# HumaticsLAB/SEAM-Match-RCNN

Hardware: AMD Instinct MI355X
Metric: video-clips/sec (10f x 800^2, 32 ROI/f, 1k gallery) (higher is better)
Workload: dtype f32; 1 GPU; configs[1] full pipeline, fixed ROIs: 10 frames 800x800 -> ResNet-50-FPN + RPN head -> RoIAlign 14x14 (32 ROI/frame) -> mask head -> match trunk x2 -> SEAM NLB + attention pool (32 seq x 10) -> pair logits vs 1000-product bank -> top-20; hip_graph=False, hip_streams=2, frames=10, rois_per_frame=32, gallery=1000, topk=20, parallelism=single GPU

## Files before the change

include/seam_hip.h:

```cpp
#ifndef SEAM_HIP_H
#define SEAM_HIP_H

#include <stdint.h>

#ifdef __cplusplus
extern "C" {
#endif

typedef void* seam_stream_t;

int seam_version(void);
int seam_fastdiv_exact(unsigned d, unsigned long long n_max);
const char* seam_error_string(int code);

int seam_option_count(void);
const char* seam_option_name(int index);
int seam_set_option(const char* name, int value);
int seam_get_option(const char* name, int* value);

int seam_conv_kred(int C, int R, int S);
int seam_conv_rows_padded(int K);
int seam_conv_tile(int M, int K);
int seam_conv_tile_prec(int prec, int M, int K);
int seam_conv_tile_taps(int prec, int M, int K, int taps);
// ... 7 lines not shown
                    int relu, seam_stream_t stream);

int seam_conv2d_upres_f32(const float* x, const float* w_packed, const float* scale, const float* shift,
                          const float* top, float* y, int N, int H, int W, int C, int K, int R, int S,
                          int stride, int pad, int Ht, int Wt, int relu, seam_stream_t stream);

int seam_conv2d_crop_f32(const float* x, const float* w_packed, const float* scale, const float* shift, float* y,
                         int N, int H, int W, int C, int K, int R, int S, int stride, int pad, int Ho, int Wo,
                         int relu, seam_stream_t stream);
int seam_conv2d_crop_f16(const void* x, const void* w_packed, const float* scale, const float* shift, void* y,
                         int N, int H, int W, int C, int K, int R, int S, int stride, int pad, int Ho, int Wo,
                         int relu, seam_stream_t stream);

int seam_conv2d_dual_f32(const float* x1, const float* x2, const float* w_packed, const float* scale,
                         const float* shift, float* y, int N, int Ho, int Wo, int C1, int H2, int W2, int C2,
                         int stride2, int K, int relu, seam_stream_t stream);

int seam_conv1x1_sw_config(int M, int C1, int C2, int K);
int seam_conv1x1_sw_f32(const float* x, const float* x2, const float* w, const float* shift, const float* residual, float* y,
                        int M, int C1, int C2, int K, int relu, int res_mode, int Ho, int Wo, int rH, int rW,
                        seam_stream_t stream);

int seam_conv1x1_f16pc_supported(long long M, int C, int K);
long long seam_conv1x1_f16pc_weight_halves(int K, int C);
int seam_pack_conv1x1_weight_f16pc(const float* w, void* w_packed, int K, int C, seam_stream_t stream);
int seam_conv1x1_f16pc(const void* x, const void* w_packed, const float* scale, const float* shift, const void* residual, void* y,
                       long long M, int C, int K, int relu, seam_stream_t stream);

int seam_conv1x1_sxpc_supported(long long M, int C, int K);
long long seam_conv1x1_sxpc_weight_bytes(int K, int C);
int seam_pack_conv1x1_weight_sxpc(const float* w, void* w_packed, int K, int C, seam_stream_t stream);
int seam_conv1x1_sxpc(const float* x, const void* w_packed, const float* scale, const float* shift, const float* residual, float* y,
                      long long M, int C, int K, int relu, seam_stream_t stream);

int seam_conv1x1_swh_config(long long M, int C1, int C2, int K);
int seam_conv1x1_swh_f16(const void* x, const void* x2, const void* w, const float* scale, const float* shift,
                         const void* residual, void* y, long long M, int C1, int C2, int K, int relu, int res_mode,
                         int Ho, int Wo, int rH, int rW, seam_stream_t stream);

int seam_stem_s2d_swh_f16(const void* xpad, const void* w, const float* scale, const float* shift, void* y, int N, int Ho, int Wo,
                          int relu, seam_stream_t stream);

int seam_conv1x1_pc_supported(long long M, int C, int K);
long long seam_conv1x1_pc_weight_floats(int K, int C);
int seam_pack_conv1x1_pc_f32(const float* w, float* w_packed, int K, int C, seam_stream_t stream);
int seam_conv1x1_pc_f32(const float* x, const float* w_packed, const float* scale, const float* shift, const float* residual,
                        float* y, long long M, int C, int K, int relu, seam_stream_t stream);

int seam_conv2d_dual_f16(const void* x1, const void* x2, const void* w_packed, const float* scale,
                         const float* shift, void* y, int N, int Ho, int Wo, int C1, int H2, int W2, int C2,
                         int stride2, int K, int relu, seam_stream_t stream);

int seam_conv_kred_f16(int C, int R, int S);
int seam_pack_conv_weight_f16(const float* w, void* w_packed, int K, int Cin, int R, int S,
                              int Cstore, int mode, seam_stream_t stream);
int seam_conv2d_f16(const void* x, const void* w_packed, const float* scale, const float* shift,
                    const void* residual, void* y, int N, int H, int W, int C, int K, int R, int S,
                    int stride, int pad, int relu, int y_f32, seam_stream_t stream);

int seam_preprocess_f32(const float* img, float* out, int in_h, int in_w, int out_h, int out_w,
                        int Hp, int Wp, seam_stream_t stream);

int seam_preprocess_f16(const float* img, void* out , int in_h, int in_w, int out_h,
                        int out_w, int Hp, int Wp, seam_stream_t stream);

int seam_preprocess_batch_f32(const float* imgs, size_t img_stride, float* out, int n, int in_h, int in_w,
// ... 341 lines not shown
```

seam-match-rcnn_amd/_native.py:

```python
from __future__ import annotations

import ctypes as C
import os

import torch

_HERE = os.path.dirname(os.path.abspath(__file__))
LIB_PATH = os.environ.get("SEAM_LIB_PATH") or os.path.join(_HERE, "lib", "libseam_hip.so")

_p = C.c_void_p
_i = C.c_int
_f = C.c_float
_i64 = C.c_int64

class TrunkLayer(C.Structure):
    _fields_ = [("w", C.c_void_p), ("u", C.c_void_p), ("u24", C.c_void_p), ("scale", C.c_void_p), ("shift", C.c_void_p)]


SGD_MAX_SLOTS = 32
SGD_FP_SLOTS = 64


class SgdTensor(C.Structure):
    _fields_ = [("p", C.c_void_p), ("g", C.c_void_p), ("buf", C.c_void_p), ("numel", C.c_int64), ("group", C.c_int), ("reserved", C.c_int)]
# ... 30 lines not shown
    "seam_set_option": (_i, [C.c_char_p, _i]),
    "seam_get_option": (_i, [C.c_char_p, C.POINTER(_i)]),
    "seam_conv_kred": (_i, [_i, _i, _i]),
    "seam_conv_rows_padded": (_i, [_i]),
    "seam_conv_tile": (_i, [_i, _i]),
    "seam_conv_tile_prec": (_i, [_i, _i, _i]),
    "seam_conv_tile_taps": (_i, [_i, _i, _i, _i]),
    "seam_pack_conv_weight_f32": (_i, [_p, _p, _i, _i, _i, _i, _i, _i, _p]),
    "seam_conv2d_f32": (_i, [_p, _p, _p, _p, _p, _p, _i, _i, _i, _i, _i, _i, _i, _i, _i, _i, _p]),
    "seam_linear_narrow_supported": (_i, [_i, _i]),
    "seam_pack_linear_narrow_f32": (_i, [_p, _p, _i, _i, _p]),
    "seam_linear_narrow_f32": (_i, [_p, _p, _p, _p, C.c_longlong, _i, _i, _i, _p]),
    "seam_conv2d_crop_f32": (_i, [_p, _p, _p, _p, _p, _i, _i, _i, _i, _i, _i, _i, _i, _i, _i, _i, _i, _p]),
    "seam_conv2d_crop_f16": (_i, [_p, _p, _p, _p, _p, _i, _i, _i, _i, _i, _i, _i, _i, _i, _i, _i, _i, _p]),
    "seam_preprocess_s2d_batch_f32": (_i, [_p, C.c_size_t, _p, _i, _i, _i, _i, _i, _i, _i, _p]),
    "seam_preprocess_s2d_batch_f16": (_i, [_p, C.c_size_t, _p, _i, _i, _i, _i, _i, _i, _i, _p]),
    "seam_preprocess_s2d_pad_batch_f16": (_i, [_p, C.c_size_t, _p, _i, _i, _i, _i, _i, _i, _i, _i, _i, _p]),
    "seam_conv2d_dual_f32": (_i, [_p, _p, _p, _p, _p, _p, _i, _i, _i, _i, _i, _i, _i, _i, _i, _i, _p]),
    "seam_conv1x1_pc_supported": (_i, [C.c_longlong, _i, _i]),
    "seam_conv1x1_pc_weight_floats": (C.c_longlong, [_i, _i]),
    "seam_pack_conv1x1_pc_f32": (_i, [_p, _p, _i, _i, _p]),
    "seam_conv1x1_pc_f32": (_i, [_p, _p, _p, _p, _p, _p, C.c_longlong, _i, _i, _i, _p]),
    "seam_conv1x1_sw_config": (_i, [_i, _i, _i, _i]),
    "seam_conv1x1_sw_f32": (_i, [_p, _p, _p, _p, _p, _p, _i, _i, _i, _i, _i, _i, _i, _i, _i, _i, _p]),
    "seam_conv1x1_swh_config": (_i, [C.c_longlong, _i, _i, _i]),
    "seam_conv1x1_f16pc_supported": (_i, [C.c_longlong, _i, _i]),
    "seam_conv1x1_f16pc_weight_halves": (C.c_longlong, [_i, _i]),
    "seam_pack_conv1x1_weight_f16pc": (_i, [_p, _p, _i, _i, _p]),
    "seam_conv1x1_f16pc": (_i, [_p, _p, _p, _p, _p, _p, C.c_longlong, _i, _i, _i, _p]),
    "seam_conv1x1_sxpc_supported": (_i, [C.c_longlong, _i, _i]),
    "seam_conv1x1_sxpc_weight_bytes": (C.c_longlong, [_i, _i]),
    "seam_pack_conv1x1_weight_sxpc": (_i, [_p, _p, _i, _i, _p]),
    "seam_conv1x1_sxpc": (_i, [_p, _p, _p, _p, _p, _p, C.c_longlong, _i, _i, _i, _p]),
    "seam_conv1x1_swh_f16": (_i, [_p, _p, _p, _p, _p, _p, _p, C.c_longlong, _i, _i, _i, _i, _i, _i, _i, _i, _i, _p]),
    "seam_stem_s2d_swh_f16": (_i, [_p, _p, _p, _p, _p, _i, _i, _i, _i, _p]),
    "seam_conv2d_dual_f16": (_i, [_p, _p, _p, _p, _p, _p, _i, _i, _i, _i, _i, _i, _i, _i, _i, _i, _p]),
    "seam_conv2d_upres_f32": (_i, [_p, _p, _p, _p, _p, _p, _i, _i, _i, _i, _i, _i, _i, _i, _i, _i, _i, _i, _p]),
    "seam_pack_conv_weight_bx3": (_i, [_p, _p, _p, _i, _i, _i, _i, _i, _i, _p]),
    "seam_conv2d_bx3": (_i, [_p, _p, _p, _p, _p, _p, _i, _i, _i, _i, _i, _i, _i, _i, _i, _i, _p]),
    "seam_pack_conv_weight_sx": (_i, [_p, _p, _p, _i, _i, _i, _i, _i, _i, _p]),
    "seam_conv2d_sx": (_i, [_p, _p, _p, _p, _p, _p, _i, _i, _i, _i, _i, _i, _i, _i, _i, _i, _i, _p]),
    "seam_wino_supported": (_i, [_i, _i, _i, _i, _i]),
    "seam_wino_weight_floats": (C.c_longlong, [_i, _i]),
    "seam_wino_slot_fill_pct": (_i, [_i, _i, _i, _i, _i, _i]),
    "seam_wino_tile_variant": (_i, [_i, _i, _i, _i, _i, _i]),
    "seam_pack_conv_weight_wino_f32": (_i, [_p, _p, _i, _i, _i, _i, _p]),
    "seam_wino_issue_slots": (C.c_longlong, [_i, _i, _i, _i, _i, _i]),
    "seam_wino24_issue_slots": (C.c_longlong, [_i, _i, _i, _i, _i, _i]),
    "seam_wino24_variant": (_i, [_i, _i, _i, _i, _i, _i]),
    "seam_wino24_form": (_i, [_i, _i, _i, _i, _i, _i]),
    "seam_wino24_weight_floats": (C.c_longlong, [_i, _i]),
    "seam_pack_conv_weight_wino24_f32": (_i, [_p, _p, _i, _i, _i, _i, _p]),
    "seam_conv3x3_wino24_f32": (_i, [_p, _p, _p, _p, _p, _p, _i, _i, _i, _i, _i, _i, _i, _p]),
    "seam_conv3x3_wino_f32": (_i, [_p, _p, _p, _p, _p, _p, _i, _i, _i, _i, _i, _i, _i, _p]),
    "seam_conv3x3_f16pc_supported": (_i, [_i, _i, _i, _i, _i, _i]),
    "seam_conv3x3_f16pc_pays": (_i, [_i, _i, _i, _i, _i, _i]),
    "seam_f16pc_weight_halves": (C.c_longlong, [_i, _i]),
    "seam_pack_conv_weight_f16pc": (_i, [_p, _p, _i, _i, _i, _p]),
    "seam_conv3x3_f16pc": (_i, [_p, _p, _p, _p, _p, _p, _i, _i, _i, _i, _i, _i, _i, _p]),
    "seam_conv_kred_f16": (_i, [_i, _i, _i]),
    "seam_pack_conv_weight_f16": (_i, [_p, _p, _i, _i, _i, _i, _i, _i, _p]),
    "seam_conv2d_f16": (_i, [_p, _p, _p, _p, _p, _p, _i, _i, _i, _i, _i, _i, _i, _i, _i, _i, _i, _p]),
    "seam_preprocess_f32": (_i, [_p, _p, _i, _i, _i, _i, _i, _i, _p]),
    "seam_preprocess_batch_f32": (_i, [_p, C.c_size_t, _p, _i, _i, _i, _i, _i, _i, _i, _p]),
    "seam_preprocess_batch_f16": (_i, [_p, C.c_size_t, _p, _i, _i, _i, _i, _i, _i, _i, _p]),
    "seam_preprocess_u8": (_i, [_p, _p, _i, _i, _i, _i, _i, _i, _i, _p]),
# ... 168 lines not shown
```

seam-match-rcnn_amd/csrc/seam_pwsx.hip:

```cpp
#include <hip/hip_runtime.h>
#include "seam_device.h"
#include <stdint.h>
#include <type_traits>
#include "seam_fastdiv.h"
#include "seam_launch.h"
#include "seam_pack_items.h"
#include "seam_split.h"

namespace {

constexpr int BM = 128;
constexpr int CK = 64;
constexpr int KS = CK / 16;
constexpr int PLB = CK * 2;
constexpr int ROWB = 3 * PLB + 16;
constexpr int ABUF = BM * ROWB;
constexpr int NP = BM * (CK / 4) / 256;
constexpr int TROW = 128 + 16;
constexpr int TBUF = 32 * TROW;
constexpr int TR0 = 2 * ABUF;
constexpr int LDS_BYTES = TR0 + 4 * 2 * TBUF;
static_assert(LDS_BYTES <= 160 * 1024 && ABUF + 3 * PLB < 65536 && 4 * 32 * ROWB < 65536, "LDS map / ds immediates");
constexpr int RB = 4;
static_assert(RB == KS, "ring slot = k-step of the chunk");
constexpr int RVA = 3;

#ifndef SEAM_SXPC_ABL
#define SEAM_SXPC_ABL 0
#endif

struct SxpcArgs {
    const float* x;
    const void* w;
    const float* scale;
    const float* shift;
    const float* res;
    float* y;
    int M, C, K, relu;
    int tiles_n, nchunks, total_tiles;
    unsigned m_tiles_n;
};

__global__ __launch_bounds__(512, 2) void conv1x1_sxpc(const SxpcArgs p) {
    extern __shared__ __attribute__((aligned(16))) char smem[];
    const int tid = threadIdx.x, lane = tid & 63;
    const int wave = __builtin_amdgcn_readfirstlane(tid >> 6);
    const bool consumer = wave < 4;
    const int n = p.nchunks;

    const XcdTiles xt = xcd_tiles(p.total_tiles);
    const int ntiles = xt.ntiles, S = xt.stride;
    if (ntiles == 0) return;
    const int tile0 = xt.tile0();
    const size_t row_bytes = (size_t)p.C * 4, out_row = (size_t)p.K * 4;
    const int total_chunks = ntiles * n;

    if (!consumer) {
        const int ptid = tid - 256;
        unsigned goff[NP];
        LDSQ char* lp[NP];
#pragma unroll
        for (int r = 0; r < NP; ++r) {
            const int row = (ptid >> 4) + 16 * r;
            goff[r] = (unsigned)(row * p.C * 4 + (ptid & 15) * 16);
            lp[r] = (LDSQ char*)smem + row * ROWB + (ptid & 15) * 8;
        }
        f32x4 rq[2][NP];
        int tile = tile0, ck = 0, tiles_left = ntiles;
        auto x_desc = [&](const int tl) {
            const int tm = fdivu(tl, p.tiles_n, p.m_tiles_n);
            const int row0 = tm * BM;
            const int rows = tiles_left > 0 ? min(BM, p.M - row0) : 0;
            return __builtin_amdgcn_make_buffer_rsrc((void*)((const char*)p.x + (size_t)(tiles_left > 0 ? row0 : 0) * row_bytes), 0,
                                                     (int)(rows * row_bytes), 0x00020000);
        };
        __amdgpu_buffer_rsrc_t rs = x_desc(tile);
        auto request = [&](f32x4 (&dst)[NP]) {
#pragma unroll
            for (int r = 0; r < NP; ++r)
                dst[r] = __builtin_bit_cast(f32x4, __builtin_amdgcn_raw_buffer_load_b128(rs, (SEAM_SXPC_ABL & 1) ? kOob : goff[r], ck * (CK * 4), 0));
            if (++ck == n) {
                ck = 0;
                tile += S;
                --tiles_left;
                rs = x_desc(tile);
            }
        };
        auto store_chunk = [&](const f32x4 (&src)[NP], const int buf) {
            if (SEAM_SXPC_ABL & 1) return;
#pragma unroll
            for (int r = 0; r < NP; ++r) {
                u32x2 q0, q1, q2;
                if (SEAM_SXPC_ABL & 4) {
                    q0[0] = __builtin_bit_cast(unsigned, src[r][0]); q0[1] = __builtin_bit_cast(unsigned, src[r][1]);
                    q1[0] = __builtin_bit_cast(unsigned, src[r][2]); q1[1] = __builtin_bit_cast(unsigned, src[r][3]); q2 = q0;
                } else {
                    split3_bf16(src[r], q0, q1, q2);
                }
                *reinterpret_cast<u32x2 LDSQ*>(lp[r] + buf * ABUF) = q0;
                *reinterpret_cast<u32x2 LDSQ*>(lp[r] + buf * ABUF + PLB) = q1;
                *reinterpret_cast<u32x2 LDSQ*>(lp[r] + buf * ABUF + 2 * PLB) = q2;
            }
        };
        request(rq[0]);
        request(rq[1]);
        store_chunk(rq[0], 0);
        request(rq[0]);
        LDS_BAR();
        for (int c = 0; c < total_chunks; c += 2) {
            store_chunk(rq[1], 1);
            request(rq[1]);
            LDS_BAR();
            if (c + 1 >= total_chunks) break;
            store_chunk(rq[0], 0);
            request(rq[0]);
            LDS_BAR();
        }
    } else {
// ... 119 lines not shown
                }
                auto put = [&](const int m) {
#pragma unroll
                    for (int qd = 0; qd < 4; ++qd)
                        *reinterpret_cast<f32x4 LDSQ*>(tw + (m & 1) * TBUF + qd * 32) =
                            f32x4{acc[m][4 * qd], acc[m][4 * qd + 1], acc[m][4 * qd + 2], acc[m][4 * qd + 3]};
                };
                put(0);
#pragma unroll
                for (int m = 0; m < 4; ++m) {
                    if (m + 1 < 4) put(m + 1);
#pragma unroll
                    for (int i = 0; i < 4; ++i) {
                        f32x4 v = *reinterpret_cast<const f32x4 LDSQ*>(tr + (m & 1) * TBUF + i * (8 * TROW));
                        v = v * sc + sh;
                        if (RES) v += rv[m][i];
                        if (RELU) {
#pragma unroll
                            for (int e = 0; e < 4; ++e) v[e] = fmaxf(v[e], 0.f);
                        }
                        __builtin_amdgcn_raw_buffer_store_b128(__builtin_bit_cast(u32x4, v), y_rsrc, ocol + m * K32 + i * K8, 0, 0);
                    }
                }
            };
            if (p.res) {
                if (p.relu) finish_tile(std::true_type{}, std::true_type{}); else finish_tile(std::true_type{}, std::false_type{});
            } else {
                if (p.relu) finish_tile(std::false_type{}, std::true_type{}); else finish_tile(std::false_type{}, std::false_type{});
            }
        }
    }
}

__global__ void sxpc_pack_kernel(const float* __restrict__ w, unsigned short* __restrict__ out, int K, int C) {
    const size_t total = (size_t)K * C / 8;
    for (size_t i = (size_t)blockIdx.x * blockDim.x + threadIdx.x; i < total; i += (size_t)gridDim.x * blockDim.x)
        seam_pack::sxpc_item(w, out, i, C);
}

int sxpc_plan(SxpcArgs& a, long long M, int C, int K) {
    if (M <= 0 || C < 256 || (C % CK) || K < 128 || (K % 128)) return 1;
    if ((unsigned long long)BM * C * 4 >= kOob || (unsigned long long)BM * K * 4 >= kOob) return 1;
    if ((unsigned long long)(C / 16) * 3072 >= kOob) return 1;
    const long long tiles_m = (M + BM - 1) / BM;
    const long long total = tiles_m * (K / 128);
    if (total >= (1LL << 24) || M >= (1LL << 31)) return 1;
    a.M = (int)M; a.C = C; a.K = K;
    a.tiles_n = K / 128; a.nchunks = C / CK; a.total_tiles = (int)total;
    if (!seam_fastdiv::exact(a.tiles_n, 2ull * total + (1ull << 16))) return 1;
    a.m_tiles_n = seam_fastdiv::magic(a.tiles_n);
    return 0;
}

}

extern "C" {

int seam_conv1x1_sxpc_supported(long long M, int C, int K) {
    SxpcArgs a;
    return sxpc_plan(a, M, C, K) == 0 ? 1 : 0;
}

long long seam_conv1x1_sxpc_weight_bytes(int K, int C) { return (long long)K * C * 6; }

int seam_pack_conv1x1_weight_sxpc(const float* w, void* w_packed, int K, int C, void* stream) {
    SxpcArgs a;
    if (sxpc_plan(a, 1, C, K)) return (int)hipErrorInvalidValue;
    const size_t total = (size_t)K * C / 8;
    const unsigned grid = seam_launch::grid256(total);
    hipLaunchKernelGGL(sxpc_pack_kernel, dim3(grid), dim3(256), 0, (hipStream_t)stream, w, (unsigned short*)w_packed, K, C);
    return (int)hipGetLastError();
}

int seam_conv1x1_sxpc(const float* x, const void* w_packed, const float* scale, const float* shift, const float* residual, float* y,
                      long long M, int C, int K, int relu, void* stream) {
    SxpcArgs a;
    if ((relu != 0 && relu != 1) || sxpc_plan(a, M, C, K)) return (int)hipErrorInvalidValue;
    a.x = x; a.w = w_packed; a.scale = scale; a.shift = shift; a.res = residual; a.y = y; a.relu = relu;
    int ncu;
    const hipError_t e = seam_launch::prepare<conv1x1_sxpc>(LDS_BYTES, &ncu);
    if (e != hipSuccess) return (int)e;
    const unsigned grid = (unsigned)(a.total_tiles > ncu ? ncu : a.total_tiles);
    hipLaunchKernelGGL(conv1x1_sxpc, dim3(grid), dim3(512), LDS_BYTES, (hipStream_t)stream, a);
    return (int)hipGetLastError();
}

}
```

seam-match-rcnn_amd/models/detection.py:

```python
from __future__ import annotations

import math
from collections import OrderedDict
from typing import List, Sequence, Tuple

import numpy as np
import torch
import torch.nn.functional as F
from torch import nn

from .. import ops

RESNET50_LAYERS = ((3, 64, 1), (4, 128, 2), (6, 256, 2), (3, 512, 2))
BBOX_XFORM_CLIP = math.log(1000.0 / 16)
NMS_MAX_BOXES = 16384


import os as _os


def _key(params, dtype=None) -> tuple:
    return tuple((p.data_ptr(), p._version) for p in params) + (dtype,)


def cdt(module):
    return getattr(module, "compute_dtype", torch.float32)


def adt(module) -> torch.dtype:
    return torch.float16 if cdt(module) == torch.float16 else torch.float32


SPLIT_F32 = _os.environ.get("SEAM_SPLIT_F32", "1") != "0"
SPLIT_DTYPE = {"6": ops.SX6, "9": ops.SX9}[_os.environ.get("SEAM_SPLIT_TERMS", "6")]
SPLIT_C3_MIN_C = 256
SPLIT_CLASSES = frozenset(c for c in _os.environ.get("SEAM_SPLIT_CLASSES", "c1,c3,c2s2").split(",") if c)


def split_on(module) -> bool:
    return (SPLIT_F32 and getattr(module, "split_f32", True) and cdt(module) == torch.float32 and not module.training
            and not torch.is_grad_enabled())


def set_split_f32(model: nn.Module, on: bool) -> nn.Module:
    for m in model.modules():
        m.split_f32 = bool(on)
    return model


def set_compute_dtype(model: nn.Module, dtype) -> nn.Module:
    if dtype not in (torch.float32, torch.float16, ops.BX3):
        raise ValueError('compute dtype must be torch.float32, torch.float16 or "bf16x3"')
    for m in model.modules():
        m.compute_dtype = dtype
    return model


def resized_size(h: int, w: int, min_size: int = 800, max_size: int = 1333) -> Tuple[int, int, float]:
    scale = min(float(min_size) / float(min(h, w)), float(max_size) / float(max(h, w)))
    return int(math.floor(float(h) * scale)), int(math.floor(float(w) * scale)), scale


class PreparedImages:

    def __init__(self, tensor, sizes, orig, padded, min_size, max_size, size_divisible, s2d):
        self.tensor, self.sizes, self.orig, self.padded = tensor, list(sizes), list(orig), tuple(padded)
        self.min_size, self.max_size, self.size_divisible, self.s2d = min_size, max_size, size_divisible, bool(s2d)

    def __len__(self):
# ... 101 lines not shown
        return self._all()

    def _pack_key(self):
        dt = cdt(self)
        return _key(self._all(), dt) + (dt == torch.float32 and SPLIT_F32 and getattr(self, "split_f32", True),)

    def packed(self):
        dt = cdt(self)
        sx = dt == torch.float32 and SPLIT_F32 and getattr(self, "split_f32", True)
        key = self._pack_key()
        if self._pk is None or key != self._pk_key:
            with torch.no_grad():
                pk = {"stem": ops.pack_conv(self.conv1.weight, None, self.bn1.tensors(), stride=2, pad=3,
                                            cstore=8 if dt == torch.float16 else 4, bn_eps=self.bn1.eps, dtype=dt)}
                if dt in (torch.float32, torch.float16):
                    def s2d_weight():
                        w8 = F.pad(self.conv1.weight.detach().to(torch.float32), (1, 0, 1, 0))
                        return w8.view(64, 3, 4, 2, 4, 2).permute(0, 3, 5, 1, 2, 4).reshape(64, 12, 4, 4).contiguous()
                    ws = ops.derived_source(s2d_weight, (self.conv1.weight,))
                    pk["stem_s2d"] = ops.pack_conv(ws, None, self.bn1.tensors(), stride=1, pad=2, cstore=12 if dt == torch.float32 else 16,
                                                   bn_eps=self.bn1.eps, wino=False, dtype=dt)
                    if dt == torch.float16 and STEM_SWH:
                        pk["stem_rows"] = F.pad(ws, (0, 0, 0, 0, 0, 4)).permute(0, 2, 3, 1).reshape(64, 256).to(torch.float16).contiguous()
                for li in range(1, 5):
                    for bi, b in enumerate(getattr(self, f"layer{li}")):
                        e = {"c1": ops.pack_conv(b.conv1.weight, None, b.bn1.tensors(), bn_eps=b.bn1.eps, dtype=dt),
                             "c2": ops.pack_conv(b.conv2.weight, None, b.bn2.tensors(), stride=b.stride, pad=1,
                                                 bn_eps=b.bn2.eps, dtype=dt),
                             "c3": ops.pack_conv(b.conv3.weight, None, b.bn3.tensors(), bn_eps=b.bn3.eps, dtype=dt)}
                        if b.downsample is not None:
                            e["ds"] = ops.pack_conv(b.downsample[0].weight, None, b.downsample[1].tensors(),
                                                    stride=b.stride, bn_eps=b.downsample[1].eps, dtype=dt)
                            if dt in (torch.float32, torch.float16) and FUSE_SHORTCUT:
                                e["c3ds"] = ops.pack_conv_dual(b.conv3.weight, b.bn3.tensors(), b.downsample[0].weight,
                                                               b.downsample[1].tensors(), bn_eps=b.bn3.eps, dtype=dt)
                        if sx:
                            if "c1" in SPLIT_CLASSES:
                                e["c1x"] = ops.pack_conv(b.conv1.weight, None, b.bn1.tensors(), bn_eps=b.bn1.eps, dtype=SPLIT_DTYPE)
                            if "c2s2" in SPLIT_CLASSES and b.stride == 2:
                                e["c2x"] = ops.pack_conv(b.conv2.weight, None, b.bn2.tensors(), stride=2, pad=1, bn_eps=b.bn2.eps,
                                                         dtype=SPLIT_DTYPE)
                            if "c3" in SPLIT_CLASSES and "c3ds" not in e and b.conv3.in_channels >= SPLIT_C3_MIN_C:
                                e["c3x"] = ops.pack_conv(b.conv3.weight, None, b.bn3.tensors(), bn_eps=b.bn3.eps, dtype=SPLIT_DTYPE)
                        pk[(li, bi)] = e
            self._pk, self._pk_key = pk, key
        return self._pk

    def forward(self, x: torch.Tensor, s2d_padded: bool = False, taped: bool = False) -> List[torch.Tensor]:
        if taped:
            return self.forward_taped(x, s2d_padded)
        pk = self.packed()
        n = x.shape[0]
        if BODY_STREAMS >= 2 and n >= 2 * BODY_STREAMS and x.is_cuda:
            cur = torch.cuda.current_stream()
            if (getattr(self, "_streams", None) is None or len(self._streams) != BODY_STREAMS
                    or self._streams[0].device != x.device):
                self._streams = [torch.cuda.Stream(device=x.device) for _ in range(BODY_STREAMS)]
            spad = 3 if s2d_padded else 0
            h1, w1 = ((x.shape[1] - spad, x.shape[2] - spad) if x.shape[-1] in (12, 16) else
                      ((x.shape[1] + 6 - 7) // 2 + 1, (x.shape[2] + 6 - 7) // 2 + 1))
            hh, ww = (h1 + 2 - 3) // 2 + 1, (w1 + 2 - 3) // 2 + 1
            outs = []
            for li, (nblk, planes, stride) in enumerate(RESNET50_LAYERS, start=1):
                if stride == 2:
                    hh, ww = (hh - 1) // 2 + 1, (ww - 1) // 2 + 1
                outs.append(torch.empty((n, hh, ww, planes * 4), dtype=x.dtype, device=x.device))
            bounds = [n * i // BODY_STREAMS for i in range(BODY_STREAMS + 1)]
            for i, st in enumerate(self._streams):
# ... 1 lines not shown
                with torch.cuda.stream(st):
                    lo, hi = bounds[i], bounds[i + 1]
                    self._run(x[lo:hi], pk, [o[lo:hi] for o in outs], s2d_padded)
            for st in self._streams:
                cur.wait_stream(st)
            return outs
        return self._run(x, pk, None, s2d_padded)

    def _stem(self, x, pk, s2d_padded=False, pool=True):
        if x.shape[-1] in (12, 16):
            streaming = ("stem_rows" in pk and x.dtype == torch.float16 and x.shape[-1] == 16
                         and (x.shape[1] - (3 if s2d_padded else 0)) * (x.shape[2] - (3 if s2d_padded else 0)) >= 128)
            if s2d_padded and not streaming:
                x = x[:, 2:-1, 2:-1].contiguous()
            if streaming:
                x = ops.stem_s2d_f16(x, pk["stem_rows"], pk["stem_s2d"].scale, pk["stem_s2d"].shift, relu=True, padded=s2d_padded)
            else:
                x = ops.conv2d(x, pk["stem_s2d"], relu=True, out_hw=(x.shape[1], x.shape[2]))
        else:
            x = ops.conv2d(x, pk["stem"], relu=True)
        return ops.maxpool2d(x, 3, 2, 1) if pool else x

    def _run(self, x, pk, outs, s2d_padded=False):
        x = self._stem(x, pk, s2d_padded)
        sx = split_on(self)
        feats = []
        for li in range(1, 5):
            nblk = len(getattr(self, f"layer{li}"))
            for bi in range(nblk):
                e = pk[(li, bi)]
                o = ops.conv2d(x, e.get("c1x", e["c1"]) if sx else e["c1"], relu=True)
                o = ops.conv2d(o, e.get("c2x", e["c2"]) if sx else e["c2"], relu=True)
                if "c3ds" in e:
                    x = ops.conv2d_dual(o, x, e["c3ds"], getattr(self, f"layer{li}")[bi].stride, relu=True)
                    continue
                idt = ops.conv2d(x, e["ds"]) if "ds" in e else x
                x = ops.conv2d(o, e.get("c3x", e["c3"]) if sx else e["c3"], relu=True, residual=idt,
                               out=outs[li - 1] if (outs is not None and bi == nblk - 1) else None)
            feats.append(x)
        return feats

    def blocks(self):
        return [(li, bi, b) for li in range(1, 5) for bi, b in enumerate(getattr(self, f"layer{li}"))]

    def forward_taped(self, x: torch.Tensor, s2d_padded: bool = False) -> List[torch.Tensor]:
        from ..autograd import BodyFunction
        if cdt(self) != torch.float32 or x.dtype != torch.float32:
            raise NotImplementedError("the training branch of the ResNet body is fp32 only: call set_compute_dtype(torch.float32)")
        stem = self.conv1.weight.requires_grad
        if stem and not self.train_stem:
            raise NotImplementedError(
                "ResNet body training: the stem of the backbone (backbone.body.conv1 and its max-pool) has no backward; freeze "
                "it with `model.backbone.body.conv1.weight.requires_grad_(False)` or build the model with "
                "trainable_backbone_layers <= 4 (layer1..layer4 may learn).  Stem training is opt-in: set `train_stem=True` "
                "(constructor keyword, or the attribute of backbone.body).")
        pk = self.packed()
        blocks = self.blocks()
        if stem:
            weights = [self.conv1.weight] + [w for _, _, b in blocks for w in block_weights(b)]
            meta = [(pk[(li, bi)], b.stride, b.downsample is not None, bi == len(getattr(self, f"layer{li}")) - 1) for li, bi, b in blocks]
            stem_fwd = (lambda f: self._stem(f, pk, s2d_padded, pool=False), pk["stem"].scale)
            return list(BodyFunction.apply(meta, stem_fwd, x, *weights))
        start = next((i for i, (_, _, b) in enumerate(blocks) if any(p.requires_grad for p in b.parameters())), len(blocks))
        with torch.no_grad():
            x = self._stem(x.detach(), pk, s2d_padded)
            feats = []
            for li, bi, b in blocks[:start]:
# ... 559 lines not shown
```

seam-match-rcnn_amd/ops.py:

```python
from __future__ import annotations

import ctypes as C
import functools
from dataclasses import dataclass
from typing import Optional, Sequence

import torch

from . import _native

F32 = torch.float32
F16 = torch.float16


def _stream() -> int:
    return torch.cuda.current_stream().cuda_stream


def _req(t: torch.Tensor, dtype=F32, name: str = "tensor") -> torch.Tensor:
    if not isinstance(t, torch.Tensor) or not t.is_cuda:
        raise _native.SeamNativeError(f"{name}: expected a tensor on the HIP device (no CPU path exists)")
    if dtype is not None and t.dtype != dtype:
        raise TypeError(f"{name}: expected {dtype}, got {t.dtype}")
    return t if t.is_contiguous() else t.contiguous()
# ... 577 lines not shown
    x, top = _req(x, F32, "x"), _req(top, F32, "top")
    n, h, w, c = x.shape
    if c != pc.Cstore:
        raise ValueError(f"conv2d_topdown: input has {c} channels, weights packed for {pc.Cstore}")
    ho = (h + 2 * pc.pad - pc.R) // pc.stride + 1
    wo = (w + 2 * pc.pad - pc.S) // pc.stride + 1
    if top.dim() != 4 or top.shape[0] != n or top.shape[3] != pc.K:
        raise ValueError("conv2d_topdown: top must be NHWC [N,Ht,Wt,K]")
    y = torch.empty((n, ho, wo, pc.K), dtype=F32, device=x.device)
    lib = _native.lib()
    sw = _sw_ok(pc, h, w) and h * w >= 64
    tr = CONV_TRACE is not None and _trace_begin(
        _sw_variant(lib, "sw", n * h * w, c, pc.K) if sw else _igemm_variant(lib, F32, n * ho * wo, pc.K),
        2.0 * n * ho * wo * pc.K * pc.R * pc.S * (pc.Cin or pc.Cstore), (n, h, w, c, pc.K, pc.R, pc.stride),
        float(4 * (x.numel() + pc.w.numel() + y.numel() + top.numel())))
    if sw:
        _sw_launch(lib, x, None, pc, top, y, n * h * w, c, 0, False, 2, ho, wo, top.shape[1], top.shape[2])
    else:
        _native.check(lib.seam_conv2d_upres_f32(_ptr(x), _ptr(pc.w), _ptr(pc.scale), _ptr(pc.shift), _ptr(top), _ptr(y),
                                                n, h, w, c, pc.K, pc.R, pc.S, pc.stride, pc.pad, top.shape[1], top.shape[2], 0,
                                                _stream()), "seam_conv2d_upres_f32")
    if tr:
        _trace_end(tr)
    return y


def pack_conv_dual(w1: torch.Tensor, bn1, w2: torch.Tensor, bn2, bn_eps: float = 1e-5, dtype=F32) -> PackedConv:
    def fold(w, bn):
        bw, bb, rm, rv = (t.detach().to(F32) for t in bn)
        sc = bw * torch.rsqrt(rv + bn_eps)
        return w.detach().to(F32).reshape(w.shape[0], -1) * sc[:, None], bb - rm * sc
    w = derived_source(lambda: torch.cat([fold(w1, bn1)[0], fold(w2, bn2)[0]], 1).contiguous(), (w1, w2))
    shift = derived_source(lambda: (fold(w1, bn1)[1] + fold(w2, bn2)[1]).contiguous(), ())
    return pack_conv(w[:, :, None, None], shift, wino=False, dtype=dtype)


def conv2d_dual(x1: torch.Tensor, x2: torch.Tensor, pc: PackedConv, stride2: int = 1, relu: bool = False) -> torch.Tensor:
    x1 = _req(x1, None, "x1")
    if pc.dtype not in (F32, F16) or pc.R != 1 or pc.S != 1:
        raise ValueError("conv2d_dual: needs fp32 / fp16 1x1 weights from pack_conv_dual")
    dt = pc.dtype
    x1, x2 = _req(x1, dt, "x1"), _req(x2, dt, "x2")
    n, ho, wo, c1 = x1.shape
    n2, h2, w2, c2 = x2.shape
    cm = 32 if dt == F32 else 64
    if n2 != n or c1 + c2 != pc.Cstore or c1 % cm or c2 % cm:
        raise ValueError(f"conv2d_dual: channel / batch mismatch (C1, C2 must be multiples of {cm} and sum to the packed width)")
    if (ho - 1) * stride2 >= h2 or (wo - 1) * stride2 >= w2:
        raise ValueError("conv2d_dual: x2 too small for the output grid")
    y = torch.empty((n, ho, wo, pc.K), dtype=dt, device=x1.device)
    lib = _native.lib()
    same = stride2 == 1 and (h2, w2) == (ho, wo)
    sw = dt == F32 and same and _sw_ok(pc, ho, wo)
    swh = dt == F16 and same and _swh_ok(pc, ho, wo) and lib.seam_conv1x1_swh_config(n * ho * wo, c1, c2, pc.K) != 0
    tr = CONV_TRACE is not None and _trace_begin(
        _sw_variant(lib, "sw" if sw else "swh", n * ho * wo, c1 + c2, pc.K) if sw or swh else _igemm_variant(lib, dt, n * ho * wo, pc.K, dual=True),
        2.0 * n * ho * wo * pc.K * (c1 + c2), (n, ho, wo, c1 + c2, pc.K, 1, 1),
        float(x1.element_size() * (x1.numel() + n * ho * wo * c2 + pc.w.numel() + y.numel())))
    if sw:
        _sw_launch(lib, x1, x2, pc, None, y, n * ho * wo, c1, c2, relu)
    elif swh:
        _native.check(lib.seam_conv1x1_swh_f16(_ptr(x1), _ptr(x2), _ptr(pc.wsh), _ptr(pc.scale), _ptr(pc.shift), None, _ptr(y),
                                               n * ho * wo, c1, c2, pc.K, 1 if relu else 0, 0, 0, 0, 0, 0, _stream()), "seam_conv1x1_swh_f16")
    else:
        fn = lib.seam_conv2d_dual_f32 if dt == F32 else lib.seam_conv2d_dual_f16
        _native.check(fn(_ptr(x1), _ptr(x2), _ptr(pc.w), _ptr(pc.scale), _ptr(pc.shift), _ptr(y), n, ho, wo, c1,
                         h2, w2, c2, stride2, pc.K, int(relu), _stream()), "seam_conv2d_dual")
    if tr:
        _trace_end(tr)
    return y


def linear(x: torch.Tensor, pc: PackedConv, relu: bool = False, out_f32: bool = False) -> torch.Tensor:
    m, c = x.shape
    return conv2d(x.view(m, 1, 1, c), pc, relu, out_f32=out_f32).view(m, pc.K)


def match_trunk(x: torch.Tensor, convs: Sequence[PackedConv], lin: PackedConv) -> torch.Tensor:
    lib = _native.lib()
    x = _req(x, F32, "x")
    k = x.shape[0]
    if tuple(x.shape[1:]) != (14, 14, 256) or len(convs) != 4 or any(pc.dtype != F32 for pc in list(convs) + [lin]):
        raise ValueError("match_trunk: fp32 NHWC [K,14,14,256] input and fp32-packed layers expected")
    out = torch.empty((k, 256), dtype=F32, device=x.device)
# ... 1690 lines not shown
```

Before: 74.24 clips/s.

## Add dual-input split-bf16 1x1 conv kernel for fused conv3+downsample shortcut

Adds a DUAL variant of the split-bf16 (SX6) pointwise conv kernel that streams the channel chunks of the main input and then the strided shortcut input, with per-tile buffer descriptors and fast-division index math. The conv3+downsample shortcut in the bottleneck blocks now packs an SX6 twin and routes through this kernel when split mode is on. Previously the fused dual conv used plain fp32 while other 1x1 convs used the split-bf16 path. The intent is to run this fused step on the faster matrix path, at the cost of extra address arithmetic and a small precision change for these layers.

Result: faster. 76.37 clips/s, median of 6 (+2.9%).

```diff
diff --git a/include/seam_hip.h b/include/seam_hip.h
--- a/include/seam_hip.h
+++ b/include/seam_hip.h
@@ -63,6 +63,10 @@
 int seam_pack_conv1x1_weight_sxpc(const float* w, void* w_packed, int K, int C, seam_stream_t stream);
 int seam_conv1x1_sxpc(const float* x, const void* w_packed, const float* scale, const float* shift, const float* residual, float* y,
                       long long M, int C, int K, int relu, seam_stream_t stream);
+
+int seam_conv1x1_sxpc_dual_supported(long long M, int C1, int C2, int K);
+int seam_conv1x1_sxpc_dual(const float* x1, const float* x2, const void* w_packed, const float* scale, const float* shift, float* y,
+                           int N, int Ho, int Wo, int C1, int H2, int W2, int C2, int stride2, int K, int relu, seam_stream_t stream);
 
 int seam_conv1x1_swh_config(long long M, int C1, int C2, int K);
 int seam_conv1x1_swh_f16(const void* x, const void* x2, const void* w, const float* scale, const float* shift,
diff --git a/seam-match-rcnn_amd/_native.py b/seam-match-rcnn_amd/_native.py
--- a/seam-match-rcnn_amd/_native.py
+++ b/seam-match-rcnn_amd/_native.py
@@ -86,6 +86,8 @@
     "seam_conv1x1_sxpc_weight_bytes": (C.c_longlong, [_i, _i]),
     "seam_pack_conv1x1_weight_sxpc": (_i, [_p, _p, _i, _i, _p]),
     "seam_conv1x1_sxpc": (_i, [_p, _p, _p, _p, _p, _p, C.c_longlong, _i, _i, _i, _p]),
+    "seam_conv1x1_sxpc_dual_supported": (_i, [C.c_longlong, _i, _i, _i]),
+    "seam_conv1x1_sxpc_dual": (_i, [_p, _p, _p, _p, _p, _p, _i, _i, _i, _i, _i, _i, _i, _i, _i, _i, _p]),
     "seam_conv1x1_swh_f16": (_i, [_p, _p, _p, _p, _p, _p, _p, C.c_longlong, _i, _i, _i, _i, _i, _i, _i, _i, _i, _p]),
     "seam_stem_s2d_swh_f16": (_i, [_p, _p, _p, _p, _p, _i, _i, _i, _i, _p]),
     "seam_conv2d_dual_f16": (_i, [_p, _p, _p, _p, _p, _p, _i, _i, _i, _i, _i, _i, _i, _i, _i, _i, _p]),
diff --git a/seam-match-rcnn_amd/csrc/seam_pwsx.hip b/seam-match-rcnn_amd/csrc/seam_pwsx.hip
--- a/seam-match-rcnn_amd/csrc/seam_pwsx.hip
+++ b/seam-match-rcnn_amd/csrc/seam_pwsx.hip
@@ -1,6 +1,7 @@
 #include <hip/hip_runtime.h>
 #include "seam_device.h"
 #include <stdint.h>
+#include <algorithm>
 #include <type_traits>
 #include "seam_fastdiv.h"
 #include "seam_launch.h"
@@ -41,7 +42,18 @@
     unsigned m_tiles_n;
 };
 
-__global__ __launch_bounds__(512, 2) void conv1x1_sxpc(const SxpcArgs p) {
+struct SxpcDual {
+    const float* x2;
+    unsigned long long img2_bytes;
+    int N, C1, n1;
+    unsigned HoWo, Wo;
+    unsigned m_howo, one_howo, thr;
+    unsigned m_wo, one_wo;
+    unsigned img_step, row_step, px_step;
+};
+
+template <bool DUAL>
+__device__ __forceinline__ void sxpc_body(const SxpcArgs& p, const SxpcDual& d) {
     extern __shared__ __attribute__((aligned(16))) char smem[];
     const int tid = threadIdx.x, lane = tid & 63;
     const int wave = __builtin_amdgcn_readfirstlane(tid >> 6);
@@ -52,7 +64,8 @@
     const int ntiles = xt.ntiles, S = xt.stride;
     if (ntiles == 0) return;
     const int tile0 = xt.tile0();
-    const size_t row_bytes = (size_t)p.C * 4, out_row = (size_t)p.K * 4;
+    const int c1 = DUAL ? d.C1 : p.C;
+    const size_t row_bytes = (size_t)c1 * 4, out_row = (size_t)p.K * 4;
     const int total_chunks = ntiles * n;
 
     if (!consumer) {
@@ -62,7 +75,7 @@
 #pragma unroll
         for (int r = 0; r < NP; ++r) {
             const int row = (ptid >> 4) + 16 * r;
-            goff[r] = (unsigned)(row * p.C * 4 + (ptid & 15) * 16);
+            goff[r] = (unsigned)(row * c1 * 4 + (ptid & 15) * 16);
             lp[r] = (LDSQ char*)smem + row * ROWB + (ptid & 15) * 8;
         }
         f32x4 rq[2][NP];
@@ -75,15 +88,43 @@
                                                      (int)(rows * row_bytes), 0x00020000);
         };
         __amdgpu_buffer_rsrc_t rs = x_desc(tile);
+        unsigned goff2[DUAL ? NP : 1];
+        __amdgpu_buffer_rsrc_t rs2;
+        auto x2_tile = [&](const int tl) {
+            const bool live = tiles_left > 0;
+            const unsigned row0 = live ? (unsigned)fdivu(tl, p.tiles_n, p.m_tiles_n) * BM : 0u;
+            const unsigned n_first = __builtin_amdgcn_readfirstlane(row0 / d.HoWo);
+            const unsigned long long left = (unsigned long long)((unsigned)d.N - n_first) * d.img2_bytes;
+            rs2 = __builtin_amdgcn_make_buffer_rsrc((void*)((const char*)d.x2 + (size_t)n_first * d.img2_bytes), 0,
+                                                    live ? (int)(left > kOob ? kOob : (unsigned)left) : 0, 0x00020000);
+            const unsigned rl0 = row0 - n_first * d.HoWo + (unsigned)(ptid >> 4);
+#pragma unroll
+            for (int r = 0; r < NP; ++r) {
+                const unsigned rl = rl0 + 16 * r;
+                const unsigned nl = __umulhi(rl, d.m_howo) + rl * d.one_howo + (rl >= d.thr ? 1u : 0u);
+                const unsigned rem = rl - nl * d.HoWo;
+                const unsigned ho = __umulhi(rem, d.m_wo) + rem * d.one_wo, wo = rem - ho * d.Wo;
+                const unsigned off = nl * d.img_step + ho * d.row_step + wo * d.px_step + (unsigned)((ptid & 15) * 16);
+                goff2[r] = row0 + (unsigned)(ptid >> 4) + 16 * r < (unsigned)p.M ? off : kOob;
+            }
+        };
+        if (DUAL) x2_tile(tile);
         auto request = [&](f32x4 (&dst)[NP]) {
-#pragma unroll
-            for (int r = 0; r < NP; ++r)
-                dst[r] = __builtin_bit_cast(f32x4, __builtin_amdgcn_raw_buffer_load_b128(rs, (SEAM_SXPC_ABL & 1) ? kOob : goff[r], ck * (CK * 4), 0));
+            if (!DUAL || ck < d.n1) {
+#pragma unroll
+                for (int r = 0; r < NP; ++r)
+                    dst[r] = __builtin_bit_cast(f32x4, __builtin_amdgcn_raw_buffer_load_b128(rs, (SEAM_SXPC_ABL & 1) ? kOob : goff[r], ck * (CK * 4), 0));
+            } else {
+#pragma unroll
+                for (int r = 0; r < NP; ++r)
+                    dst[r] = __builtin_bit_cast(f32x4, __builtin_amdgcn_raw_buffer_load_b128(rs2, (SEAM_SXPC_ABL & 1) ? kOob : goff2[r], (ck - d.n1) * (CK * 4), 0));
+            }
             if (++ck == n) {
                 ck = 0;
                 tile += S;
                 --tiles_left;
                 rs = x_desc(tile);
+                if (DUAL) x2_tile(tile);
             }
         };
         auto store_chunk = [&](const f32x4 (&src)[NP], const int buf) {
@@ -269,6 +310,9 @@
     }
 }
 
+__global__ __launch_bounds__(512, 2) void conv1x1_sxpc(const SxpcArgs p) { sxpc_body<false>(p, SxpcDual{}); }
+__global__ __launch_bounds__(512, 2) void conv1x1_sxpc_dual(const SxpcArgs p, const SxpcDual d) { sxpc_body<true>(p, d); }
+
 __global__ void sxpc_pack_kernel(const float* __restrict__ w, unsigned short* __restrict__ out, int K, int C) {
     const size_t total = (size_t)K * C / 8;
     for (size_t i = (size_t)blockIdx.x * blockDim.x + threadIdx.x; i < total; i += (size_t)gridDim.x * blockDim.x)
@@ -289,6 +333,33 @@
     return 0;
 }
 
+int sxpc_dual_plan(SxpcArgs& a, SxpcDual& d, long long N, long long Ho, long long Wo, int C1, long long H2, long long W2, int C2, int stride2, int K) {
+    if (N <= 0 || Ho <= 0 || Wo <= 0 || H2 <= 0 || W2 <= 0 || C1 < CK || C2 < CK || (C1 % CK) || (C2 % CK) || stride2 < 1) return 1;
+    if (N >= (1LL << 31) || Ho >= (1LL << 31) || Wo >= (1LL << 31) || H2 >= (1LL << 31) || W2 >= (1LL << 31)) return 1;
+    if ((Ho - 1) * stride2 >= H2 || (Wo - 1) * stride2 >= W2) return 1;
+    if (Ho * Wo >= (1LL << 31) || N * (Ho * Wo) >= (1LL << 31)) return 1;
+    if (sxpc_plan(a, N * Ho * Wo, C1 + C2, K)) return 1;
+    const long long HoWo = Ho * Wo;
+    if ((unsigned long long)H2 * W2 >= (1ull << 31) / ((unsigned long long)C2 * 4)) return 1;
+    const unsigned long long img2 = (unsigned long long)H2 * W2 * C2 * 4;
+    const unsigned long long imgs = std::min<unsigned long long>((unsigned long long)N, (unsigned long long)((BM - 2) / HoWo + 2));
+    if (imgs * img2 > kOob) return 1;
+    const bool mid = HoWo >= 2 && HoWo < BM;
+    if (mid && !seam_fastdiv::exact((unsigned long long)HoWo, (unsigned long long)(BM + HoWo))) return 1;
+    if (!seam_fastdiv::exact((unsigned long long)Wo, (unsigned long long)HoWo)) return 1;
+    d.img2_bytes = img2;
+    d.N = (int)N; d.C1 = C1; d.n1 = C1 / CK; d.HoWo = (unsigned)HoWo; d.Wo = (unsigned)Wo;
+    d.m_howo = mid ? seam_fastdiv::magic((unsigned long long)HoWo) : 0u;
+    d.one_howo = HoWo == 1 ? 1u : 0u;
+    d.thr = HoWo >= BM ? (unsigned)HoWo : 0xffffffffu;
+    d.m_wo = seam_fastdiv::magic((unsigned long long)Wo);
+    d.one_wo = Wo == 1 ? 1u : 0u;
+    d.img_step = (unsigned)img2;
+    d.row_step = (unsigned)((unsigned long long)stride2 * W2 * C2 * 4);
+    d.px_step = (unsigned)((unsigned long long)stride2 * C2 * 4);
+    return 0;
+}
+
 }
 
 extern "C" {
@@ -322,4 +393,25 @@
     return (int)hipGetLastError();
 }
 
-}
+int seam_conv1x1_sxpc_dual_supported(long long M, int C1, int C2, int K) {
+    SxpcArgs a;
+    if (C1 < CK || C2 < CK || (C1 % CK) || (C2 % CK) || (long long)C1 + C2 >= (1LL << 30)) return 0;
+    return sxpc_plan(a, M, C1 + C2, K) == 0 ? 1 : 0;
+}
+
+int seam_conv1x1_sxpc_dual(const float* x1, const float* x2, const void* w_packed, const float* scale, const float* shift, float* y,
+                           int N, int Ho, int Wo, int C1, int H2, int W2, int C2, int stride2, int K, int relu, void* stream) {
+    SxpcArgs a;
+    SxpcDual d;
+    if ((relu != 0 && relu != 1) || !x2 || sxpc_dual_plan(a, d, N, Ho, Wo, C1, H2, W2, C2, stride2, K)) return (int)hipErrorInvalidValue;
+    a.x = x1; a.w = w_packed; a.scale = scale; a.shift = shift; a.res = nullptr; a.y = y; a.relu = relu;
+    d.x2 = x2;
+    int ncu;
+    const hipError_t e = seam_launch::prepare<conv1x1_sxpc_dual>(LDS_BYTES, &ncu);
+    if (e != hipSuccess) return (int)e;
+    const unsigned grid = (unsigned)(a.total_tiles > ncu ? ncu : a.total_tiles);
+    hipLaunchKernelGGL(conv1x1_sxpc_dual, dim3(grid), dim3(512), LDS_BYTES, (hipStream_t)stream, a, d);
+    return (int)hipGetLastError();
+}
+
+}
diff --git a/seam-match-rcnn_amd/models/detection.py b/seam-match-rcnn_amd/models/detection.py
--- a/seam-match-rcnn_amd/models/detection.py
+++ b/seam-match-rcnn_amd/models/detection.py
@@ -34,7 +34,8 @@
 SPLIT_F32 = _os.environ.get("SEAM_SPLIT_F32", "1") != "0"
 SPLIT_DTYPE = {"6": ops.SX6, "9": ops.SX9}[_os.environ.get("SEAM_SPLIT_TERMS", "6")]
 SPLIT_C3_MIN_C = 256
-SPLIT_CLASSES = frozenset(c for c in _os.environ.get("SEAM_SPLIT_CLASSES", "c1,c3,c2s2").split(",") if c)
+SPLIT_C3DS_MIN_C = 384
+SPLIT_CLASSES = frozenset(c for c in _os.environ.get("SEAM_SPLIT_CLASSES", "c1,c3,c2s2,c3ds").split(",") if c)
 
 
 def split_on(module) -> bool:
@@ -202,8 +203,13 @@
                             e["ds"] = ops.pack_conv(b.downsample[0].weight, None, b.downsample[1].tensors(),
                                                     stride=b.stride, bn_eps=b.downsample[1].eps, dtype=dt)
                             if dt in (torch.float32, torch.float16) and FUSE_SHORTCUT:
-                                e["c3ds"] = ops.pack_conv_dual(b.conv3.weight, b.bn3.tensors(), b.downsample[0].weight,
-                                                               b.downsample[1].tensors(), bn_eps=b.bn3.eps, dtype=dt)
+                                twin = (sx and "c3ds" in SPLIT_CLASSES and SPLIT_DTYPE == ops.SX6
+                                        and b.conv3.in_channels + b.downsample[0].in_channels >= SPLIT_C3DS_MIN_C)
+                                packs = ops.pack_conv_dual(b.conv3.weight, b.bn3.tensors(), b.downsample[0].weight, b.downsample[1].tensors(),
+                                                           bn_eps=b.bn3.eps, dtype=(dt, ops.SX6) if twin else (dt,))
+                                e["c3ds"] = packs[0]
+                                if twin:
+                                    e["c3dsx"] = packs[1]
                         if sx:
                             if "c1" in SPLIT_CLASSES:
                                 e["c1x"] = ops.pack_conv(b.conv1.weight, None, b.bn1.tensors(), bn_eps=b.bn1.eps, dtype=SPLIT_DTYPE)
@@ -271,7 +277,7 @@
                 o = ops.conv2d(x, e.get("c1x", e["c1"]) if sx else e["c1"], relu=True)
                 o = ops.conv2d(o, e.get("c2x", e["c2"]) if sx else e["c2"], relu=True)
                 if "c3ds" in e:
-                    x = ops.conv2d_dual(o, x, e["c3ds"], getattr(self, f"layer{li}")[bi].stride, relu=True)
+                    x = ops.conv2d_dual(o, x, e.get("c3dsx", e["c3ds"]) if sx else e["c3ds"], getattr(self, f"layer{li}")[bi].stride, relu=True)
                     continue
                 idt = ops.conv2d(x, e["ds"]) if "ds" in e else x
                 x = ops.conv2d(o, e.get("c3x", e["c3"]) if sx else e["c3"], relu=True, residual=idt,
diff --git a/seam-match-rcnn_amd/ops.py b/seam-match-rcnn_amd/ops.py
--- a/seam-match-rcnn_amd/ops.py
+++ b/seam-match-rcnn_amd/ops.py
@@ -633,24 +633,43 @@
         return w.detach().to(F32).reshape(w.shape[0], -1) * sc[:, None], bb - rm * sc
     w = derived_source(lambda: torch.cat([fold(w1, bn1)[0], fold(w2, bn2)[0]], 1).contiguous(), (w1, w2))
     shift = derived_source(lambda: (fold(w1, bn1)[1] + fold(w2, bn2)[1]).contiguous(), ())
+    if isinstance(dtype, tuple):
+        return tuple(pack_conv(w[:, :, None, None], shift, wino=False, dtype=d) for d in dtype)
     return pack_conv(w[:, :, None, None], shift, wino=False, dtype=dtype)
+
+
+def _sxpc_dual_map_ok(n, ho, wo, h2, w2, c2) -> bool:
+    return 4 * h2 * w2 * c2 * min(n, 126 // (ho * wo) + 2) <= 1 << 31 and ho * wo * wo < 1 << 32
 
 
 def conv2d_dual(x1: torch.Tensor, x2: torch.Tensor, pc: PackedConv, stride2: int = 1, relu: bool = False) -> torch.Tensor:
     x1 = _req(x1, None, "x1")
-    if pc.dtype not in (F32, F16) or pc.R != 1 or pc.S != 1:
-        raise ValueError("conv2d_dual: needs fp32 / fp16 1x1 weights from pack_conv_dual")
-    dt = pc.dtype
+    if pc.dtype not in (F32, F16, SX6) or pc.R != 1 or pc.S != 1:
+        raise ValueError("conv2d_dual: needs fp32 / fp16 / split-bf16 (SX6) 1x1 weights from pack_conv_dual")
+    dt = F32 if pc.dtype == SX6 else pc.dtype
     x1, x2 = _req(x1, dt, "x1"), _req(x2, dt, "x2")
     n, ho, wo, c1 = x1.shape
     n2, h2, w2, c2 = x2.shape
     cm = 32 if dt == F32 else 64
     if n2 != n or c1 + c2 != pc.Cstore or c1 % cm or c2 % cm:
         raise ValueError(f"conv2d_dual: channel / batch mismatch (C1, C2 must be multiples of {cm} and sum to the packed width)")
-    if (ho - 1) * stride2 >= h2 or (wo - 1) * stride2 >= w2:
+    if stride2 < 1 or (ho - 1) * stride2 >= h2 or (wo - 1) * stride2 >= w2:
         raise ValueError("conv2d_dual: x2 too small for the output grid")
+    lib = _native.lib()
+    if pc.dtype == SX6:
+        if (SXPC and pc.wx is not None and relu in (0, 1, False, True) and lib.seam_conv1x1_sxpc_dual_supported(n * ho * wo, c1, c2, pc.K) == 1
+                and _sxpc_dual_map_ok(n, ho, wo, h2, w2, c2)):
+            y = torch.empty((n, ho, wo, pc.K), dtype=F32, device=x1.device)
+            tr = CONV_TRACE is not None and _trace_begin(
+                "conv1x1_sxpc_dual", 2.0 * n * ho * wo * pc.K * (c1 + c2), (n, ho, wo, c1 + c2, pc.K, 1, 1),
+                float(x1.element_size() * (x1.numel() + n * ho * wo * c2 + pc.K * (c1 + c2) + y.numel())))
+            _native.check(lib.seam_conv1x1_sxpc_dual(_ptr(x1), _ptr(x2), _ptr(pc.wx), _ptr(pc.scale), _ptr(pc.shift), _ptr(y), n, ho, wo, c1,
+                                                     h2, w2, c2, stride2, pc.K, 1 if relu else 0, _stream()), "seam_conv1x1_sxpc_dual")
+            if tr:
+                _trace_end(tr)
+            return y
+        return conv2d(torch.cat([x1, x2[:, :(ho - 1) * stride2 + 1:stride2, :(wo - 1) * stride2 + 1:stride2]], -1), pc, relu=relu)
     y = torch.empty((n, ho, wo, pc.K), dtype=dt, device=x1.device)
-    lib = _native.lib()
     same = stride2 == 1 and (h2, w2) == (ho, wo)
     sw = dt == F32 and same and _sw_ok(pc, ho, wo)
     swh = dt == F16 and same and _swh_ok(pc, ho, wo) and lib.seam_conv1x1_swh_config(n * ho * wo, c1, c2, pc.K) != 0
```
